# barrust/pyprobables

Hardware: AMD Instinct MI355X
Metric: million keys/sec insert+lookup (Bloom m=2^28 k=7, CMS 2^20x5) (higher is better)
Workload: dtype u64; 1 GPU; cfg2 Bloom m=2^28 k=7: per rank per step clear + insert 10M 16B keys + (merge) + check them; keys_per_rank=10000000, key_bytes=16, m_bits=268435456, k=7, parallelism=single GPU

## Files before the change

pyprobables_amd/csrc/psk_capi.hip:

```cpp
#include "psk_host.hpp"

#include <map>
#include <mutex>
#include <utility>

static thread_local char g_err[512] = "";

int fail(int code, const char *fmt, ...)
{
    va_list ap;
    va_start(ap, fmt);
    vsnprintf(g_err, sizeof(g_err), fmt, ap);
    va_end(ap);
    return code;
}


extern "C" const char *psk_last_error(void) { return g_err; }
extern "C" int psk_version(void) { return 100; }

extern "C" int psk_device_count(int *count)
{
    if (!count) return fail(PSK_EINVAL, "count is NULL");
    int n = 0;
// ... 444 lines not shown
    s->opt[d->ho] = value;
    return PSK_OK;
}

extern "C" int psk_sketch_get_option(psk_sketch *s, const char *name, int64_t *value)
{
    if (!s || !name || !value) return fail(PSK_EINVAL, "NULL argument");
    if (!strcmp(name, "table_private")) {
        *value = s->table_private ? 1 : 0;
        return PSK_OK;
    }
    if (!strcmp(name, "window_pending_batches")) {
        *value = s->win.n ? (int64_t)s->win.batches.size() : 0;
        return PSK_OK;
    }
    const OptDesc *d = opt_find(name);
    if (!d || d->ho < 0) return fail(PSK_EINVAL, "%s is not a per-sketch option", name);
    *value = s->opt[d->ho] != kHoUnset ? s->opt[d->ho] : __atomic_load_n(d->var, __ATOMIC_RELAXED);
    return PSK_OK;
}

extern "C" int psk_get_option(const char *name, int64_t *value)
{
    if (!name || !value) return fail(PSK_EINVAL, "NULL argument");
    const OptDesc *d = opt_find(name);
    if (!d) return fail(PSK_EINVAL, "unknown option %s", name);
    *value = __atomic_load_n(d->var, __ATOMIC_RELAXED);
    return PSK_OK;
}

// ... 33 lines not shown
```

pyprobables_amd/csrc/psk_host.hpp:

```cpp
#pragma once
#include "psk_device.hpp"
#include "psk_partition.hpp"
#include "psk_part_bins.hpp"

#include <hip/hip_runtime.h>

#include <cstdarg>
#include <cstdio>
#include <cstdlib>
#include <cstring>
#include <new>
#include <type_traits>
#include <vector>

#include "../../include/psk.h"

using namespace psk;

#define PSK_HIDDEN __attribute__((visibility("hidden")))

PSK_HIDDEN int fail(int code, const char *fmt, ...);

#define HIP_TRY(expr)                                                                                   \
    do {                                                                                                \
// ... 201 lines not shown
                               uint64_t max_buckets = kPartMaxBuckets, int target_lg = 8)
{
    if (cells >= (1ULL << 32) || cells < (1ULL << 16)) return false;
    const uint32_t lg = 63 - __builtin_clzll(cells);
    int shift = (int)lg - target_lg;
    if (shift > (int)max_shift) shift = max_shift;
    if (shift < (int)min_shift) shift = min_shift;
    const uint64_t B = (cells + (1ULL << shift) - 1) >> shift;
    if (B > max_buckets) return false;
    g->nbuckets = (uint32_t)B;
    g->shift = (uint32_t)shift;
    g->dbg = (uint32_t)g_part_debug | (g_ragged_sort == 0 ? kGeomNoSortBit : 0u);
    g->split = g->split_idx = 0;
    g->dense = 0;
    g->append = 0;
    return true;
}

static inline bool nib_geometry(uint64_t cells, bool update, PartGeom *g)
{
    if (update ? cells <= (1ULL << g_nib_min_lg_update) : cells < (1ULL << g_nib_min_lg_lookup)) return false;
    return part_slices(cells, kNibShift, 15, g, kPartMaxBuckets, 8);
}

static inline bool nib_load_ok(uint64_t n, uint32_t k, uint64_t cells) { return n * (uint64_t)k * 2 <= cells * 5; }

static inline bool scat_geometry(const psk_sketch *s, uint64_t cap, PartGeom *g)
{
    if (!nib_geometry(s->m, true, g)) return false;
    g->k = s->k;
// ... 101 lines not shown
        tk = ((n + nwg * tiles_per_wg - 1) / (nwg * tiles_per_wg) + 63) & ~63ULL;
        if (tk > tile_full) tk = tile_full;
    }
    const double mean = (double)tiles_per_wg * (double)tk * kk / (double)g->nbuckets;
    uint64_t segcap = (uint64_t)(mean / 6.0 + 0.5 * (double)tiles_per_wg + 8.0 * __builtin_sqrt(mean) / 6.0 + 16.0);
    if constexpr (pay_tile_tag<Pay>::value) {
        if (tiles_per_wg > 16) return fail(PSK_EINVAL, "lookup round of %llu keys needs %llu tiles per workgroup (max 16)",
                                           (unsigned long long)n, (unsigned long long)tiles_per_wg);
    }
    if (segcap >= (1u << 24) || (uint64_t)g->nbuckets * segcap >= (1ULL << 32))
        return fail(PSK_EINVAL, "partition round of %llu keys is too large (segments of %llu groups)", (unsigned long long)n, (unsigned long long)segcap);
    g->nwg = (uint32_t)nwg;
    g->segcap = (uint32_t)segcap;
    g->tile = (uint32_t)tk;
    g->dense = (mean / 6.0 + 0.5 * (double)tiles_per_wg) < (double)g_part_dense_groups ? 1u : 0u;
    PSK_TRY(ensure(s->s_part, (uint64_t)g->nbuckets * nwg * segcap * 16 + 256));
    PSK_TRY(ensure(s->s_cnt, (uint64_t)g->nbuckets * nwg * 4 + 128));
    auto kern = k_part_bins<Src, IdxFn, Pay, Spill, KT, kBinKpt>;
    PSK_TRY(set_dyn_lds(kern, bp.lds));
    hipLaunchKernelGGL(kern, dim3((unsigned)nwg), dim3(kBinThreads), bp.lds, st, src, idxfn, pay, spill, *g, (uint32_t)n, bp.cap, bp.stride,
                       (uint32_t *)s->s_cnt.p, (uint4 *)s->s_part.p);
    HIP_TRY(hipGetLastError());
    return PSK_OK;
}
template <class Src, class IdxFn, class Pay, class Spill, int KT, int NT>
static int launch_scatter_nt(psk_sketch *s, const Src &src, const IdxFn &idxfn, const Pay &pay, const Spill &spill, PartGeom *g,
                             uint64_t n, hipStream_t st, uint32_t want_wgs, const ScatterTarget *fixed = nullptr)
{
    if constexpr (bins_eligible<Src, Pay, KT>::value) {
        BinsPlan bp;
// ... 40 lines not shown
        if (tk > tile_full) tk = tile_full;
    }
    const size_t lds = scatter_lds_bytes<Pay, KT, NT>(g, tk, kSorted);
    const double mean = (double)tiles_per_wg * (double)tk * kk / (double)g->nbuckets;
    uint64_t segcap = (uint64_t)(mean / Tile::GS + 0.5 * (double)tiles_per_wg + 8.0 * __builtin_sqrt(mean) / Tile::GS + 16.0);
    if constexpr (Pay::mode == kModeKeyed || pay_tile_tag<Pay>::value) {
        if (tiles_per_wg > 16) return fail(PSK_EINVAL, "lookup round of %llu keys needs %llu tiles per workgroup (max 16)",
                                           (unsigned long long)n, (unsigned long long)tiles_per_wg);
    }
    if (segcap >= (1u << 24) || (uint64_t)g->nbuckets * segcap >= (1ULL << 32))
        return fail(PSK_EINVAL, "partition round of %llu keys is too large (segments of %llu groups)", (unsigned long long)n, (unsigned long long)segcap);
    g->nwg = (uint32_t)nwg;
    g->segcap = (uint32_t)segcap;
    g->tile = (uint32_t)tk;
    g->dense = (mean / Tile::GS + 0.5 * (double)tiles_per_wg) < (double)g_part_dense_groups ? 1u : 0u;
    PSK_TRY(ensure(s->s_part, (uint64_t)g->nbuckets * nwg * segcap * 16 + 256));
    PSK_TRY(ensure(s->s_cnt, (uint64_t)g->nbuckets * nwg * 4 + 128));
    auto kern = k_part_scatter<Src, IdxFn, Pay, Spill, KT, NT>;
    PSK_TRY(set_dyn_lds(kern, lds));
    hipLaunchKernelGGL(kern, dim3((unsigned)nwg), dim3(NT), lds, st, src, idxfn, pay, spill, *g, n, (uint32_t *)s->s_cnt.p,
                       (uint4 *)s->s_part.p);
    HIP_TRY(hipGetLastError());
    return PSK_OK;
}


template <class Pay, int KT, bool FAT = true>
static int scatter_threads(const PartGeom *g)
{
    if constexpr (!FAT && (pay_fat512<Pay>::value || pay_fat1024<Pay>::value)) return scatter_threads<PaySlim<Pay>, KT, false>(g);
// ... 233 lines not shown
```

pyprobables_amd/csrc/psk_part_bins.hpp:

```cpp
#pragma once
#include "psk_partition.hpp"

namespace psk {

#ifndef PSK_BINS_NT
#define PSK_BINS_NT 768
#endif
constexpr int kBinThreads = PSK_BINS_NT;
constexpr int kBinMinWaves = kBinThreads <= 512 ? 4 : (kBinThreads <= 768 ? 6 : 8);
#ifndef PSK_BINS_KPT
#define PSK_BINS_KPT 2
#endif
constexpr int kBinKpt = PSK_BINS_KPT;
constexpr int kBinSlicesPerLane = 2;

template <class Pay>
struct pay_bins_ok { static constexpr bool value = false; };
template <>
struct pay_bins_ok<PayNone> { static constexpr bool value = true; };
template <>
struct pay_bins_ok<PayTileTag> { static constexpr bool value = true; };
template <>
struct pay_bins_ok<PayWeightSmall> { static constexpr bool value = true; };

constexpr uint32_t kBinHead = 2;
template <bool WP>
__device__ __forceinline__ uint4 bin_short_group(const uint2 a0, const uint2 a1, const uint2 a2, uint32_t nv, uint32_t mask, uint32_t t0, uint32_t t1)
{
    uint32_t f[6] = {a0.x, a0.y, a1.x, a1.y, a2.x, a2.y};
#pragma unroll
    for (int x = 1; x < 6; ++x)
        if ((uint32_t)x >= nv) f[x] = WP ? 0u : mask;
    const uint32_t n0 = nv < 3u ? nv : 3u, n1 = nv - n0;
    uint4 o;
    o.x = f[0] | (f[1] << 20);
    o.y = (f[1] >> 12) | (f[2] << 8) | ((n0 | t0) << 28);
    o.z = f[3] | (f[4] << 20);
    o.w = (f[4] >> 12) | (f[5] << 8) | ((n1 | t1) << 28);
    return o;
}
template <class Src, class IdxFn, class Pay, class Spill, int KT, int KPT>
__global__ __launch_bounds__(kBinThreads, kBinMinWaves) void k_part_bins(Src src, IdxFn idxfn, Pay pay, Spill spill, PartGeom g, uint32_t n, uint32_t cap,
                                                              uint32_t stride, uint32_t *segcnt, uint4 *buckets)
{
    constexpr int NT = kBinThreads;
    extern __shared__ __attribute__((aligned(16))) uint32_t smem[];
    char *lds = reinterpret_cast<char *>(smem);
    const uint32_t B = g.nbuckets;
    constexpr bool kExactK = KT != 8;
    const uint32_t k = kExactK ? (uint32_t)KT : g.k;
    const uint32_t mask = (1u << g.shift) - 1;
    const uint32_t tk = g.tile;
    const uint32_t ntiles = (n + tk - 1) / tk;
    const uint32_t last = n ? n - 1 : 0;
    const uint32_t stride4 = stride * 4u;
    const uint32_t lg_slices = 31u - (uint32_t)__builtin_clz(B);
    const uint32_t full4 = (cap + kBinHead) * 4u;
    constexpr uint32_t kCnt = 4;

    uint32_t L = 1;
    while (2 * L * B <= (uint32_t)NT) L *= 2;
    constexpr int kSlicesPerLane = kBinSlicesPerLane;
    const uint32_t sub = B <= (uint32_t)NT ? threadIdx.x % L : 0u;
    uint32_t myb[kSlicesPerLane], cur[kSlicesPerLane];
    uint32_t carry[kSlicesPerLane];
    uint4 *seg[kSlicesPerLane];
// ... 160 lines not shown
            const uint32_t ngroups = whole + (tail ? 1u : 0u);
            uint2 *e = reinterpret_cast<uint2 *>(bin + kBinHead * 4u);
            uint4 *out = seg[s] + cur[s];
            if (cur[s] + ngroups <= g.segcap) {
                const uint32_t hi0 = (3u | t0) << 28, hi1 = (3u | t1) << 28;
                for (uint32_t gq = sub; gq < whole; gq += L) {
                    const uint2 a0 = e[3 * gq], a1 = e[3 * gq + 1], a2 = e[3 * gq + 2];
                    uint4 o;
                    o.x = a0.x | (a0.y << 20);
                    o.y = (a0.y >> 12) | (a1.x << 8) | hi0;
                    o.z = a1.y | (a2.x << 20);
                    o.w = (a2.x >> 12) | (a2.y << 8) | hi1;
                    if (!(dbg & 1)) out[gq] = o;
                }
                if constexpr (pay_tile_tag<Pay>::value) {
                    if (tail && sub == 0 && !(dbg & 1)) out[0] = bin_short_group<WP>(e[0], e[1], e[2], rem, mask, t0, t1);
                }
                if (rem && whole && sub == (whole & (L - 1))) {
                    __builtin_amdgcn_wave_barrier();
                    const uint2 a0 = e[3 * whole], a1 = e[3 * whole + 1], a2 = e[3 * whole + 2];
                    e[0] = a0;
                    e[1] = a1;
                    e[2] = a2;
                }
                carry[s] = tail ? 0u : rem;
                cur[s] += ngroups;
            } else {
                const uint32_t nall = whole + (rem ? 1u : 0u);
                for (uint32_t gq = sub; gq < nall; gq += L) {
                    const uint2 a0 = e[3 * gq], a1 = e[3 * gq + 1], a2 = e[3 * gq + 2];
                    const uint32_t left = c - 6u * gq, nv = left < 6u ? left : 6u;
                    if (cur[s] + gq < g.segcap) {
                        out[gq] = bin_short_group<WP>(a0, a1, a2, nv, mask, t0, t1);
                    } else {
                        const uint32_t f[6] = {a0.x, a0.y, a1.x, a1.y, a2.x, a2.y};
#pragma unroll
                        for (int x = 0; x < 6; ++x)
                            if ((uint32_t)x < nv) {
                                if constexpr (pay_tile_tag<Pay>::value) {
                                    spill((b << g.shift) | f[x], tile);
                                    if (ordinal) spill((b << g.shift) | f[x], tile - gridDim.x);
                                } else if constexpr (WP) spill((b << g.shift) | (f[x] & mask), f[x] >> 15);
                                else spill((b << g.shift) | f[x], 0u);
                            }
                    }
                }
                carry[s] = 0;
                cur[s] += nall;
// ... 7 lines not shown
            Src::pin(kcur[q]);
            if constexpr (WP) asm volatile("" : "+v"(wcur[q]));
        }
        PSK_BIN_TICK(2);
        lds_barrier();
        PSK_BIN_TICK(3);
    }
    if (ordinal != ~0u) {
        const uint32_t t0 = pay_tile_tag<Pay>::value ? (ordinal & 3u) << 2 : 0u, t1 = pay_tile_tag<Pay>::value ? ordinal & 12u : 0u;
#pragma unroll
        for (int s = 0; s < kSlicesPerLane; ++s) {
            if (myb[s] == ~0u || sub != 0 || carry[s] == 0) continue;
            const uint2 *e = reinterpret_cast<const uint2 *>(lds + myb[s] * stride4 + kBinHead * 4u);
            const uint2 a0 = e[0], a1 = e[1], a2 = e[2];
            if (cur[s] < g.segcap) {
                if (!(dbg & 1)) seg[s][cur[s]] = bin_short_group<WP>(a0, a1, a2, carry[s], mask, t0, t1);
            } else {
                const uint32_t f[6] = {a0.x, a0.y, a1.x, a1.y, a2.x, a2.y};
#pragma unroll
                for (int x = 0; x < 6; ++x)
                    if ((uint32_t)x < carry[s]) {
                        if constexpr (pay_tile_tag<Pay>::value) spill((myb[s] << g.shift) | f[x], ordinal * gridDim.x + blockIdx.x);
                        else if constexpr (WP) spill((myb[s] << g.shift) | (f[x] & mask), f[x] >> 15);
                        else spill((myb[s] << g.shift) | f[x], 0u);
                    }
            }
            cur[s] += 1;
        }
    }
    if (t_lane) {
        unsigned long long *prof = reinterpret_cast<unsigned long long *>(segcnt + (size_t)g.nbuckets * g.nwg);
// ... 33 lines not shown
```

pyprobables_amd/csrc/psk_part_bloom_check.hip:

```cpp
#include "psk_host.hpp"
#include "psk_lookup.hpp"

static inline uint32_t keyed_wgs(const PartGeom &g) { return g.nbuckets >= 2048 ? 1024u : 0u; }

static int check_round_scatter(psk_sketch *s, const Batch &sub, uint64_t cnt, uint8_t *out, uint32_t *defer, PartGeom *g,
                               hipStream_t st, bool *handled)
{
    return with_part_source(sub, handled, [&](auto src) {
        using Src = decltype(src);
        return with_kt<Src>(s->k, [&](auto kt) {
            constexpr int KT = decltype(kt)::value;
            SpillBloomTest spill{(const uint32_t *)s->table, out, defer};
            return launch_scatter<Src, IdxBloom<kTuPow2>, PayKeyId, SpillBloomTest, KT>(s, src, IdxBloom<kTuPow2>{s->md}, PayKeyId{},
                                                                                         spill, g, cnt, st, keyed_wgs(*g));
        });
    });
}

static int check_round_test(psk_sketch *s, const PartGeom &g, uint8_t *out, hipStream_t st, unsigned long long *miss_ctr = nullptr)
{
    const size_t lds = (size_t)1 << (g.shift - 3);
    PSK_TRY(set_dyn_lds(k_bloom_test, lds));
    hipLaunchKernelGGL(k_bloom_test, dim3(g.nbuckets), dim3(kApplyThreads), lds, st, (const uint32_t *)s->table, s->padded_bytes / 4, g,
                       (const uint32_t *)s->s_cnt.p, (const uint4 *)s->s_part.p, out, miss_ctr);
// ... 106 lines not shown
                    }
                }
                s->tflag_wgs = want;
                return (int)PSK_OK;
            });
        }) != PSK_OK || !handled || cap == 0) return false;
    if (round_keys > cap) {
        const uint64_t rounds = (b.n + cap - 1) / cap;
        round_keys = ((b.n + rounds - 1) / rounds + 4095) & ~4095ULL;
        if (round_keys > cap) round_keys = cap;
    }
    *round_keys_out = round_keys;
    return true;
}

static uint32_t *tflag_base(psk_sketch *s) { return (uint32_t *)s->s_tflag.p + 4; }
constexpr uint32_t kResolveWgs = 256;

static int tile_flag_scatter(psk_sketch *s, const Batch &sub, uint64_t cnt, bool defer, PartGeom *g, uint32_t *gen_out, hipStream_t st, bool *handled)
{
    return with_part_source(sub, handled, [&](auto src) {
        using Src = decltype(src);
        return with_kt<Src>(s->k, [&](auto kt) {
            constexpr int KT = decltype(kt)::value;
            const uint64_t flag_bytes = (cnt / 64 + 2048) * 4 + 16;
            if (flag_bytes > s->s_tflag.cap || s->tflag_gen == 0xFFFFFFFFu) {
                PSK_TRY(ensure(s->s_tflag, flag_bytes));
                HIP_TRY(hipMemsetAsync(s->s_tflag.p, 0, s->s_tflag.cap, st));
                s->tflag_gen = 0;
            }
            const uint32_t gen = ++s->tflag_gen;
            *gen_out = gen;
            SpillBloomFlag spill{(const uint32_t *)s->table, tflag_base(s), gen, defer ? 1u : 0u};
            return launch_scatter<Src, IdxBloom<kTuPow2>, PayTileTag, SpillBloomFlag, KT>(s, src, IdxBloom<kTuPow2>{s->md}, PayTileTag{}, spill, g, cnt, st,
                                                                                          s->tflag_wgs);
        });
    });
}

static int tile_flag_test(psk_sketch *s, const Batch &sub, uint64_t cnt, const PartGeom &g, uint32_t gen, uint8_t *out, unsigned long long publish_units, hipStream_t st)
{
    bool handled = false;
    PSK_TRY(with_part_source(sub, &handled, [&](auto src) {
        using Src = decltype(src);
        uint32_t *tflag = tflag_base(s);
        const size_t lds = (size_t)1 << (g.shift - 3);
        PSK_TRY(set_dyn_lds(k_bloom_test_flag, lds));
        hipLaunchKernelGGL(k_bloom_test_flag, dim3(g.nbuckets), dim3(kApplyThreads), lds, st, (const uint32_t *)s->table, s->padded_bytes / 4, g,
                           (const uint32_t *)s->s_cnt.p, (const uint4 *)s->s_part.p, tflag, gen, s->lk.dev, out, cnt);
        HIP_TRY(hipGetLastError());
        const uint64_t ntiles = (cnt + g.tile - 1) / g.tile;
        LookupPublish pub;
        if (publish_units && s->eff[HO_BLOOM_LOOKUP] == 2 && s->lk.dev) pub = LookupPublish{s->lk.dev, s->lk.pin, publish_units, 3};
        hipLaunchKernelGGL((k_bloom_flag_resolve<Src, kTuPow2>), dim3((unsigned)(ntiles < kResolveWgs ? ntiles : kResolveWgs)), dim3(kResolveThreads), 0, st, src,
                           (const uint32_t *)s->table, s->md, s->k, (const uint32_t *)tflag, gen, g.tile, cnt, out, pub);
        HIP_TRY(hipGetLastError());
        return (int)PSK_OK;
    }));
    return handled ? (int)PSK_OK : fail(PSK_EHIP, "tile-flag lookup: layout lost its partitioned instantiation");
}

static int bloom_check_tile_flags(psk_sketch *s, const Batch &b, uint8_t *out_dev, hipStream_t st, bool *done)
{
    *done = false;
    PartGeom g;
    uint64_t round_keys = 0;
    if (!tile_flag_geometry(s, b, &g, &round_keys)) return PSK_OK;
    for (uint64_t start = 0; start < b.n; start += round_keys) {
// ... 74 lines not shown
            else
                hipLaunchKernelGGL((k_bloom_check_lazy<Src, true, false>), grid, block, 0, st, src, (const uint32_t *)s->table, s->md, s->k, b.n, out_dev, ctr);
        } else {
            hipLaunchKernelGGL((k_bloom_check_lazy<Src, false, false>), grid, block, 0, st, src, (const uint32_t *)s->table, s->md, s->k, b.n, out_dev, ctr);
        }
        HIP_TRY(hipGetLastError());
        return (int)PSK_OK;
    }));
    *done = handled;
    return PSK_OK;
}

static int choose_scheme(psk_sketch *s, hipStream_t st)
{
    if (s->eff[HO_BLOOM_LOOKUP] != 2) return (int)s->eff[HO_BLOOM_LOOKUP];
    if (!s->lk.dev) {
        HIP_TRY(hipMalloc((void **)&s->lk.dev, 8));
        void *pin = nullptr;
        HIP_TRY(hipHostMalloc(&pin, 64, hipHostMallocDefault));
        s->lk.pin = (volatile unsigned long long *)pin;
        for (int e = 0; e < 8; ++e) s->lk.pin[e] = 0;
        HIP_TRY(hipMemsetAsync(s->lk.dev, 0, 8, st));
    }
    const unsigned long long miss = s->lk.pin[0], units = s->lk.pin[1], by = s->lk.pin[2], seq = s->lk.pin[3];
    if (units) {
        const double f = (double)miss / (double)units;
        const bool clean_call = by == 1 ? f == 0.0 : f <= 1e-6;
        if (seq != s->lk.seen_seq) {
            s->lk.seen_seq = seq;
            s->lk.clean = clean_call ? s->lk.clean + 1 : 0;
        }
        const bool flags_ok = clean_call && s->lk.clean >= 2;
        const double kLazyStay = s->m <= (1ULL << 29) ? 1.6 : (s->m <= (1ULL << 30) ? 2.2 : 3.0);
        const double kLazyEnter = s->m <= (1ULL << 29) ? 0.93 : (s->m <= (1ULL << 30) ? 0.85 : 0.72);
        constexpr uint32_t kLazyBackoff = 32;
        volatile unsigned long long &lazy_seq = s->lk.pin[4], &lazy_wait = s->lk.pin[5];
        if (seq != lazy_seq) {
            lazy_seq = seq;
// ... 124 lines not shown
```

pyprobables_amd/csrc/psk_partition.hpp:

```cpp
#pragma once
#include <type_traits>
#include "psk_device.hpp"

#ifndef PSK_BENCH_KNOBS
#define PSK_BENCH_KNOBS 0
#endif

namespace psk {

constexpr bool kBenchKnobs = PSK_BENCH_KNOBS != 0;
constexpr int kPartThreads = 512;
constexpr int kPartProbes = 32;
constexpr int kPartMaxBuckets = 2048;
constexpr int kPartScanPerThread = 4;
constexpr bool kPartPipeline = true;
constexpr bool kPartHash32 = true;
constexpr uint32_t kNibShift = 18;
constexpr uint32_t kGeomNoSortBit = 0x40000000u;
constexpr int kSortSub = 16;
constexpr int kSortBins = 64 * kSortSub;
constexpr uint32_t kPadProbe = 0xFFFFFFFFu;
#ifndef PSK_EXP_PRIO
#define PSK_EXP_PRIO 1
#endif

enum PartMode { kModePlain = 0, kModeInline = 1, kModeKeyed = 2 };

struct PartGeom {
    uint32_t nbuckets;
    uint32_t shift;
    uint32_t nwg;
    uint32_t segcap;
    uint32_t k;
    uint32_t tile;
    uint32_t dbg;
    uint32_t split;
    uint32_t split_idx;
    uint32_t dense;
    uint32_t append;
};

__device__ __forceinline__ uint64_t seg_index(const PartGeom &g, uint32_t b, uint32_t wg) { return (uint64_t)wg * g.nbuckets + b; }

template <bool POW2>
struct IdxBloom {
    static constexpr bool lo32 = POW2 && kPartHash32;
    Mod md;
    __device__ __forceinline__ uint32_t operator()(uint32_t, uint64_t h) const
    {
        return POW2 ? (uint32_t)reduce<true>(md, h) : reduce_small(md, h);
    }
    __device__ __forceinline__ uint32_t from32(uint32_t, uint32_t h) const { return h & (uint32_t)md.mask; }
};
template <bool POW2>
// ... 243 lines not shown
struct SpillBloomFlag {
    const uint32_t *tab;
    uint32_t *tileflag;
    uint32_t gen;
    uint32_t defer;
    __device__ __forceinline__ void operator()(uint32_t idx, uint32_t tile) const
    {
        if (defer || ((tab[idx >> 5] >> (idx & 31)) & 1u) == 0) {
            tileflag[tile] = gen;
            tileflag[-1] = gen;
        }
    }
};

__device__ __forceinline__ void lds_barrier() { asm volatile("s_waitcnt lgkmcnt(0)\n\ts_barrier" ::: "memory"); }

__device__ __forceinline__ uint32_t wave_inclusive_scan(uint32_t x)
{
    x += (uint32_t)__builtin_amdgcn_update_dpp(0, (int)x, 0x111, 0xf, 0xf, false);
    x += (uint32_t)__builtin_amdgcn_update_dpp(0, (int)x, 0x112, 0xf, 0xf, false);
    x += (uint32_t)__builtin_amdgcn_update_dpp(0, (int)x, 0x114, 0xf, 0xf, false);
    x += (uint32_t)__builtin_amdgcn_update_dpp(0, (int)x, 0x118, 0xf, 0xf, false);
    x += (uint32_t)__builtin_amdgcn_update_dpp(0, (int)x, 0x142, 0xa, 0xf, false);
    x += (uint32_t)__builtin_amdgcn_update_dpp(0, (int)x, 0x143, 0xc, 0xf, false);
    return x;
}

template <int NT>
__device__ __forceinline__ uint32_t block_exclusive_scan(uint32_t v, uint32_t *wave_tot , uint32_t *total)
{
// ... 711 lines not shown
#pragma unroll
                for (int x = 0; x < GS; ++x)
                    if (v[x] != kPadProbe) spill((slice << g2.shift) | (v[x] & mask), v[x] >> g1.shift);
            }
        }
        __syncthreads();
    }
    if (threadIdx.x < S) {
        const uint32_t slice = (c << sub_bits) + threadIdx.x;
        if (slice < g2.nbuckets) segcnt2[(uint64_t)slice * g2.nwg + p] = cur[threadIdx.x] < g2.segcap ? cur[threadIdx.x] : g2.segcap;
    }
}

constexpr int kApplyThreads = 1024;
constexpr int kApplyWaves = kApplyThreads / 64;

__device__ __forceinline__ uint32_t lane_segment_count(const uint32_t *segcnt, const PartGeom &g, uint32_t b)
{
    const uint32_t lane = threadIdx.x & 63, wave = threadIdx.x >> 6;
    const uint32_t S = g.split > 1 ? g.split : 1, s0 = g.split > 1 ? g.split_idx : 0;
    const uint32_t mine_total = g.nwg > s0 ? (g.nwg - s0 + S - 1) / S : 0;
    const uint32_t nseg = mine_total > wave ? (mine_total - wave + kApplyWaves - 1) / kApplyWaves : 0;
    return lane < nseg ? segcnt[(uint64_t)b * g.nwg + s0 + S * (wave + kApplyWaves * lane)] : 0u;
}

template <int D, class Body>
__device__ __forceinline__ void for_each_batch_at(const uint4 *buckets, const uint32_t *segcnt, const PartGeom &g, uint32_t b,
                                                  const uint4 pad, Body body, uint32_t mycnt_pre = ~0u)
{
    const uint32_t lane = threadIdx.x & 63, wave = threadIdx.x >> 6;
    const uint32_t S = g.split > 1 ? g.split : 1, s0 = g.split > 1 ? g.split_idx : 0;
    const uint32_t mycnt = mycnt_pre != ~0u ? mycnt_pre : lane_segment_count(segcnt, g, b);
    if (g.dense) {
        const uint32_t incl = wave_inclusive_scan(mycnt), excl = incl - mycnt;
        const uint32_t T = (uint32_t)__builtin_amdgcn_readlane((int)incl, 63);
        for (uint32_t G0 = 0; G0 < T; G0 += 64u * D) {
            uint4 q[D];
            uint64_t at[D];
            uint32_t wg[D];
#pragma unroll
            for (int d = 0; d < D; ++d) {
// ... 12 lines not shown
                }
                seg = seg < 64 ? seg : 63;
                wg[d] = s0 + S * (wave + kApplyWaves * seg);
                q[d] = pad;
                at[d] = ~0ULL;
                if (G < T) {
                    const uint64_t idx = seg_index(g, b, wg[d]) * g.segcap + (G - first);
                    q[d] = buckets[idx];
                    at[d] = idx;
                }
            }
            body(q, at, wg);
        }
        return;
    }
    const uint32_t chunks = (mycnt + 63) >> 6;
    const uint32_t incl = wave_inclusive_scan(chunks), excl = incl - chunks;
    const uint32_t C = (uint32_t)__builtin_amdgcn_readlane((int)incl, 63);
    for (uint32_t c0 = 0; c0 < C; c0 += D) {
        uint4 q[D];
        uint64_t at[D];
        uint32_t wg[D];
#pragma unroll
        for (int d = 0; d < D; ++d) {
            const uint32_t cc = c0 + d;
            const uint32_t seg = (uint32_t)__builtin_popcountll(__ballot(incl <= cc));
            const uint32_t sl = seg < 64 ? seg : 63;
            const uint32_t v = (cc - (uint32_t)__builtin_amdgcn_readlane((int)excl, sl)) * 64 + lane;
            const uint32_t cnt = seg < 64 ? (uint32_t)__builtin_amdgcn_readlane((int)mycnt, sl) : 0;
            wg[d] = s0 + S * (wave + kApplyWaves * sl);
            const uint64_t base = seg_index(g, b, wg[d]) * g.segcap;
            q[d] = pad;
            at[d] = ~0ULL;
            if (v < cnt) {
                q[d] = buckets[base + v];
                at[d] = base + v;
            }
        }
        body(q, at, wg);
    }
}

template <int D, class Body>
__device__ __forceinline__ void for_each_batch(const uint4 *buckets, const uint32_t *segcnt, const PartGeom &g, uint32_t b,
                                               const uint4 pad, Body body)
{
    const uint32_t lane = threadIdx.x & 63, wave = threadIdx.x >> 6;
    const uint32_t nseg = g.nwg > wave ? (g.nwg - wave + kApplyWaves - 1) / kApplyWaves : 0;
    uint32_t mycnt = 0;
    if (lane < nseg) mycnt = segcnt[(uint64_t)b * g.nwg + wave + kApplyWaves * lane];
    if (g.dense) {
        const uint32_t incl = wave_inclusive_scan(mycnt), excl = incl - mycnt;
        const uint32_t T = (uint32_t)__builtin_amdgcn_readlane((int)incl, 63);
        for (uint32_t G0 = 0; G0 < T; G0 += 64u * D) {
            uint4 q[D];
#pragma unroll
            for (int d = 0; d < D; ++d) {
                const uint32_t row = G0 + 64u * (uint32_t)d;
// ... 5 lines not shown
                for (; t < 64; ++t) {
                    const uint32_t end_t = (uint32_t)__builtin_amdgcn_readlane((int)incl, t);
                    if (end_t > row + 63u) break;
                    const bool past = G >= end_t;
                    seg = past ? t + 1 : seg;
                    first = past ? end_t : first;
                }
                seg = seg < 64 ? seg : 63;
                q[d] = pad;
                if (G < T) q[d] = buckets[seg_index(g, b, wave + kApplyWaves * seg) * g.segcap + (G - first)];
            }
            body(q);
        }
        return;
    }
    const uint32_t chunks = (mycnt + 63) >> 6;
    const uint32_t incl = wave_inclusive_scan(chunks), excl = incl - chunks;
    const uint32_t C = (uint32_t)__builtin_amdgcn_readlane((int)incl, 63);
    for (uint32_t c0 = 0; c0 < C; c0 += D) {
        uint4 q[D];
#pragma unroll
        for (int d = 0; d < D; ++d) {
            const uint32_t cc = c0 + d;
            const uint32_t seg = (uint32_t)__builtin_popcountll(__ballot(incl <= cc));
            const uint32_t sl = seg < 64 ? seg : 63;
            const uint32_t v = (cc - (uint32_t)__builtin_amdgcn_readlane((int)excl, sl)) * 64 + lane;
            const uint32_t cnt = seg < 64 ? (uint32_t)__builtin_amdgcn_readlane((int)mycnt, sl) : 0;
            const uint4 *src = buckets + seg_index(g, b, wave + kApplyWaves * sl) * g.segcap;
            q[d] = pad;
            if (v < cnt) q[d] = src[v];
        }
        body(q);
    }
}

constexpr int kApplyDepth = 12;

constexpr uint64_t kNtTableWords = 1ULL << 25;
__device__ __forceinline__ uint4 slice_piece(const uint32_t *tab, uint64_t tab_words, uint64_t w0, uint32_t w, bool nt = false)
{
    const uint64_t gw = w0 + w;
    if (gw + 3 < tab_words) {
        if (nt) {
            typedef unsigned int nt_u32x4 __attribute__((ext_vector_type(4)));
            const nt_u32x4 v = __builtin_nontemporal_load(reinterpret_cast<const nt_u32x4 *>(tab + gw));
// ... 15 lines not shown
    for (uint32_t wb = threadIdx.x * 4; wb < slice_words; wb += kApplyThreads * 4 * kSliceLoads) {
        uint4 t[kSliceLoads];
#pragma unroll
        for (int u = 0; u < kSliceLoads; ++u) {
            const uint32_t w = wb + (uint32_t)u * kApplyThreads * 4;
            t[u] = w < slice_words ? slice_piece(tab, tab_words, w0, w, nt) : make_uint4(0, 0, 0, 0);
        }
#pragma unroll
        for (int u = 0; u < kSliceLoads; ++u) {
            const uint32_t w = wb + (uint32_t)u * kApplyThreads * 4;
            if (w < slice_words) *reinterpret_cast<uint4 *>(smem + w) = t[u];
        }
    }
}

template <int DEPTH = kApplyDepth, class F4>
__device__ __forceinline__ void for_each_group(const uint4 *buckets, const uint32_t *segcnt, const PartGeom &g, uint32_t b,
                                               const uint4 pad, F4 f4)
{
    for_each_batch<DEPTH>(buckets, segcnt, g, b, pad, [&](const uint4 (&q)[DEPTH]) {
#pragma unroll
        for (int d = 0; d < DEPTH; ++d) f4(q[d]);
    });
}

template <class Pre, class Post>
__device__ __forceinline__ void for_each_group_padded(const uint4 *buckets, const uint32_t *segcnt, const PartGeom &g, uint32_t b,
                                                      const uint4 pad, Pre pre, Post post)
{
    for_each_batch<kApplyDepth>(buckets, segcnt, g, b, pad, [&](const uint4 (&q)[kApplyDepth]) {
        uint4 w[kApplyDepth];
#pragma unroll
        for (int d = 0; d < kApplyDepth; ++d) w[d] = pre(q[d]);
#pragma unroll
        for (int d = 0; d < kApplyDepth; ++d) post(q[d], w[d]);
// ... 4 lines not shown
constexpr uint32_t kBloomApplyCtrSpilled = 7;
struct BloomApplyStore {
    uint32_t on = 0;
    const uint32_t *spill = nullptr;
    uint32_t spill_cap = 0;
    long long *ctr = nullptr;
};
static __global__ __launch_bounds__(kApplyThreads) void k_bloom_apply(uint32_t *tab, uint64_t tab_words, PartGeom g,
                                                               const uint32_t *segcnt, const uint4 *buckets, BloomApplyStore sm)
{
    extern __shared__ __attribute__((aligned(16))) uint32_t smem[];
    const uint32_t b = blockIdx.x;
    const uint32_t slice_words = 1u << (g.shift - 5);
    for (uint32_t w = threadIdx.x; w < slice_words; w += kApplyThreads) smem[w] = 0;
    __syncthreads();
    auto half = [&](uint32_t lo, uint32_t hi) {
        const unsigned long long h = ((unsigned long long)hi << 32) | lo;
        const uint32_t nv = hi >> 28;
        if (nv > 0) { const uint32_t x = (uint32_t)h & 0xFFFFFu; atomicOr(&smem[x >> 5], 1u << (x & 31)); }
        if (nv > 1) { const uint32_t x = (uint32_t)(h >> 20) & 0xFFFFFu; atomicOr(&smem[x >> 5], 1u << (x & 31)); }
        if (nv > 2) { const uint32_t x = (uint32_t)(h >> 40) & 0xFFFFFu; atomicOr(&smem[x >> 5], 1u << (x & 31)); }
    };
    for_each_group(buckets, segcnt, g, b, make_uint4(0, 0, 0, 0), [&](const uint4 q) { half(q.x, q.y); half(q.z, q.w); });
    uint32_t spilled = 0;
    if (sm.on) {
        spilled = sm.spill[0];
        const uint32_t nsp = spilled < sm.spill_cap ? spilled : sm.spill_cap;
        const uint32_t lmask = (1u << g.shift) - 1u;
        for (uint32_t i = threadIdx.x; i < nsp; i += kApplyThreads) {
            const uint32_t x = sm.spill[2 + i];
            if ((x >> g.shift) == b) atomicOr(&smem[(x & lmask) >> 5], 1u << (x & 31));
        }
    }
    __syncthreads();
    const uint64_t w0 = (uint64_t)b * slice_words;
    const bool nt = tab_words >= kNtTableWords;
    typedef unsigned int nt_u32x4 __attribute__((ext_vector_type(4)));
    if (sm.on) {
// ... 72 lines not shown
static __global__ __launch_bounds__(kApplyThreads) void k_bloom_test(const uint32_t *tab, uint64_t tab_words, PartGeom g,
                                                              const uint32_t *segcnt, const uint4 *buckets, uint8_t *out,
                                                              unsigned long long *miss_ctr)
{
    uint32_t nmiss = 0;
    extern __shared__ __attribute__((aligned(16))) uint32_t smem[];
    const uint32_t b = blockIdx.x;
    const uint32_t slice_words = 1u << (g.shift - 5);
    const uint32_t mask = (1u << g.shift) - 1;
    const uint64_t w0 = (uint64_t)b * slice_words;
    const uint32_t dbg = kBenchKnobs ? g.dbg : 0u;
    const uint32_t mycnt = lane_segment_count(segcnt, g, b);
    if (!(dbg & 128)) load_slice(smem, tab, tab_words, w0, slice_words);
    __syncthreads();
    const uint32_t kmask = (1u << (31 - g.shift)) - 1;
    for_each_batch_at<kApplyDepth>(buckets, segcnt, g, b, make_uint4(0, 0, 0, 0), [&](const uint4 (&q)[kApplyDepth], const uint64_t (&at)[kApplyDepth],
                                                                                     const uint32_t (&wg)[kApplyDepth]) {
        uint4 w[kApplyDepth];
#pragma unroll
        for (int d = 0; d < kApplyDepth; ++d) {
            if (dbg & 64) { w[d] = make_uint4(~0u, ~0u, ~0u, ~0u); continue; }
            w[d] = make_uint4(smem[(q[d].x & mask) >> 5], smem[(q[d].y & mask) >> 5], smem[(q[d].z & mask) >> 5], smem[(q[d].w & mask) >> 5]);
        }
#pragma unroll
        for (int d = 0; d < kApplyDepth; ++d) {
            const bool live = at[d] != ~0ULL;
            const bool mx = live && ((w[d].x >> (q[d].x & 31)) & 1u) == 0;
            const bool my = live && ((w[d].y >> (q[d].y & 31)) & 1u) == 0;
            const bool mz = live && ((w[d].z >> (q[d].z & 31)) & 1u) == 0;
            const bool mw = live && ((w[d].w >> (q[d].w & 31)) & 1u) == 0;
            nmiss += (uint32_t)mx + (uint32_t)my + (uint32_t)mz + (uint32_t)mw;
            if (mx | my | mz | mw) {
                const uint32_t ordinal = (q[d].x >> 31) | ((q[d].y >> 31) << 1) | ((q[d].z >> 31) << 2) | ((q[d].w >> 31) << 3);
                const uint32_t kbase = (ordinal * g.nwg + wg[d]) * g.tile;
                if (mx) out[kbase + ((q[d].x >> g.shift) & kmask)] = 0;
                if (my) out[kbase + ((q[d].y >> g.shift) & kmask)] = 0;
                if (mz) out[kbase + ((q[d].z >> g.shift) & kmask)] = 0;
// ... 32 lines not shown
            uint4 *mid = reinterpret_cast<uint4 *>(out + (m0 - a0));
            for (uint64_t i = lo + threadIdx.x; i < hi; i += kApplyThreads) mid[i] = ones;
            if (b == 0) {
                if (threadIdx.x < (uint32_t)(m0 - a0)) out[threadIdx.x] = 1;
                if (threadIdx.x < (uint32_t)(a1 - m1)) out[(m1 - a0) + threadIdx.x] = 1;
            }
        } else if (b == 0) {
            for (uint64_t i = threadIdx.x; i < n; i += kApplyThreads) out[i] = 1;
        }
    }
    const uint32_t slice_words = 1u << (g.shift - 5);
    const uint64_t w0 = (uint64_t)b * slice_words;
    const uint32_t mycnt = lane_segment_count(segcnt, g, b);
    load_slice(smem, tab, tab_words, w0, slice_words);
    __syncthreads();
    for_each_batch_at<kFlagDepth>(buckets, segcnt, g, b, make_uint4(0, 0, 0, 0), [&](const uint4 (&q)[kFlagDepth], const uint64_t (&)[kFlagDepth],
                                                                                   const uint32_t (&wg)[kFlagDepth]) {
        uint32_t f[kFlagDepth][6], w[kFlagDepth][6];
#pragma unroll
        for (int d = 0; d < kFlagDepth; ++d) {
            f[d][0] = q[d].x & 0xFFFFFu;
            f[d][1] = __builtin_amdgcn_alignbit(q[d].y, q[d].x, 20) & 0xFFFFFu;
            f[d][2] = (q[d].y >> 8) & 0xFFFFFu;
            f[d][3] = q[d].z & 0xFFFFFu;
            f[d][4] = __builtin_amdgcn_alignbit(q[d].w, q[d].z, 20) & 0xFFFFFu;
            f[d][5] = (q[d].w >> 8) & 0xFFFFFu;
#pragma unroll
            for (int e = 0; e < 6; ++e) w[d][e] = smem[f[d][e] >> 5];
        }
#pragma unroll
        for (int d = 0; d < kFlagDepth; ++d) {
            uint32_t clear = 0;
#pragma unroll
            for (int e = 0; e < 6; ++e) clear |= (((w[d][e] >> (f[d][e] & 31)) & 1u) ^ 1u) << e;
            const uint32_t n0 = (q[d].y >> 28) & 3u, n1 = (q[d].w >> 28) & 3u;
            const uint32_t valid = ((1u << n0) - 1u) | (((1u << n1) - 1u) << 3);
            clear &= valid;
            if (clear) {
                nmiss += (uint32_t)__builtin_popcount(clear);
                const uint32_t ordinal = (q[d].y >> 30) | ((q[d].w >> 30) << 2);
                tileflag[ordinal * g.nwg + wg[d]] = gen;
                if (ordinal) tileflag[(ordinal - 1u) * g.nwg + wg[d]] = gen;
                tileflag[-1] = gen;
            }
        }
    }, mycnt);
    if (miss_ctr) {
        for (int o = 32; o > 0; o >>= 1) nmiss += __shfl_down(nmiss, o);
        __syncthreads();
        if ((threadIdx.x & 63) == 0) smem[threadIdx.x >> 6] = nmiss;
        __syncthreads();
        if (threadIdx.x == 0) {
            unsigned long long t = 0;
            for (int w = 0; w < kApplyWaves; ++w) t += smem[w];
            if (t) atomicAdd(miss_ctr, t);
        }
    }
}

constexpr int kResolveThreads = 1024;
struct LookupPublish {
// ... 218 lines not shown
```

Before: 61130 Mkeys/s.

## Pad short Bloom groups with duplicate fields and use raw LDS addressing in apply/flag kernels

Short partitioned groups are now padded by repeating their first valid field instead of a masked sentinel when the geometry flag allows it. This lets the bloom OR and flag-check kernels apply all six fields branch-free and test membership with a single AND across the fields, skipping per-field validity masks. LDS accesses are rewritten as raw address-space-3 byte offsets, with a trap that asserts dynamic LDS starts at zero, and wave indices are made scalar via readfirstlane to simplify segment base addressing. Lookup tally allocation is also made unconditional so miss counts are always published and exposed as a queryable option, which adds a small allocation and publish cost.

```diff
diff --git a/pyprobables_amd/csrc/psk_capi.hip b/pyprobables_amd/csrc/psk_capi.hip
--- a/pyprobables_amd/csrc/psk_capi.hip
+++ b/pyprobables_amd/csrc/psk_capi.hip
@@ -482,6 +482,10 @@
         *value = s->win.n ? (int64_t)s->win.batches.size() : 0;
         return PSK_OK;
     }
+    if (!strcmp(name, "bloom_lookup_misses")) {
+        *value = s->lk.pin && s->lk.pin[1] ? (int64_t)s->lk.pin[0] : -1;
+        return PSK_OK;
+    }
     const OptDesc *d = opt_find(name);
     if (!d || d->ho < 0) return fail(PSK_EINVAL, "%s is not a per-sketch option", name);
     *value = s->opt[d->ho] != kHoUnset ? s->opt[d->ho] : __atomic_load_n(d->var, __ATOMIC_RELAXED);
diff --git a/pyprobables_amd/csrc/psk_host.hpp b/pyprobables_amd/csrc/psk_host.hpp
--- a/pyprobables_amd/csrc/psk_host.hpp
+++ b/pyprobables_amd/csrc/psk_host.hpp
@@ -239,6 +239,7 @@
     g->split = g->split_idx = 0;
     g->dense = 0;
     g->append = 0;
+    g->dup_pads = 0;
     return true;
 }
 
@@ -370,6 +371,7 @@
     g->segcap = (uint32_t)segcap;
     g->tile = (uint32_t)tk;
     g->dense = (mean / 6.0 + 0.5 * (double)tiles_per_wg) < (double)g_part_dense_groups ? 1u : 0u;
+    g->dup_pads = (std::is_same<Pay, PayNone>::value && std::is_same<Spill, SpillBloomOr>::value) || pay_tile_tag<Pay>::value ? 1u : 0u;
     PSK_TRY(ensure(s->s_part, (uint64_t)g->nbuckets * nwg * segcap * 16 + 256));
     PSK_TRY(ensure(s->s_cnt, (uint64_t)g->nbuckets * nwg * 4 + 128));
     auto kern = k_part_bins<Src, IdxFn, Pay, Spill, KT, kBinKpt>;
@@ -440,6 +442,7 @@
     g->segcap = (uint32_t)segcap;
     g->tile = (uint32_t)tk;
     g->dense = (mean / Tile::GS + 0.5 * (double)tiles_per_wg) < (double)g_part_dense_groups ? 1u : 0u;
+    g->dup_pads = 0;
     PSK_TRY(ensure(s->s_part, (uint64_t)g->nbuckets * nwg * segcap * 16 + 256));
     PSK_TRY(ensure(s->s_cnt, (uint64_t)g->nbuckets * nwg * 4 + 128));
     auto kern = k_part_scatter<Src, IdxFn, Pay, Spill, KT, NT>;
diff --git a/pyprobables_amd/csrc/psk_part_bins.hpp b/pyprobables_amd/csrc/psk_part_bins.hpp
--- a/pyprobables_amd/csrc/psk_part_bins.hpp
+++ b/pyprobables_amd/csrc/psk_part_bins.hpp
@@ -25,12 +25,13 @@
 
 constexpr uint32_t kBinHead = 2;
 template <bool WP>
-__device__ __forceinline__ uint4 bin_short_group(const uint2 a0, const uint2 a1, const uint2 a2, uint32_t nv, uint32_t mask, uint32_t t0, uint32_t t1)
+__device__ __forceinline__ uint4 bin_short_group(const uint2 a0, const uint2 a1, const uint2 a2, uint32_t nv, uint32_t mask, uint32_t t0, uint32_t t1, bool dup)
 {
     uint32_t f[6] = {a0.x, a0.y, a1.x, a1.y, a2.x, a2.y};
+    const uint32_t fill = WP ? 0u : (dup ? f[0] : mask);
 #pragma unroll
     for (int x = 1; x < 6; ++x)
-        if ((uint32_t)x >= nv) f[x] = WP ? 0u : mask;
+        if ((uint32_t)x >= nv) f[x] = fill;
     const uint32_t n0 = nv < 3u ? nv : 3u, n1 = nv - n0;
     uint4 o;
     o.x = f[0] | (f[1] << 20);
@@ -50,6 +51,7 @@
     constexpr bool kExactK = KT != 8;
     const uint32_t k = kExactK ? (uint32_t)KT : g.k;
     const uint32_t mask = (1u << g.shift) - 1;
+    const bool dup = g.dup_pads != 0;
     const uint32_t tk = g.tile;
     const uint32_t ntiles = (n + tk - 1) / tk;
     const uint32_t last = n ? n - 1 : 0;
@@ -240,7 +242,7 @@
                     if (!(dbg & 1)) out[gq] = o;
                 }
                 if constexpr (pay_tile_tag<Pay>::value) {
-                    if (tail && sub == 0 && !(dbg & 1)) out[0] = bin_short_group<WP>(e[0], e[1], e[2], rem, mask, t0, t1);
+                    if (tail && sub == 0 && !(dbg & 1)) out[0] = bin_short_group<WP>(e[0], e[1], e[2], rem, mask, t0, t1, dup);
                 }
                 if (rem && whole && sub == (whole & (L - 1))) {
                     __builtin_amdgcn_wave_barrier();
@@ -257,7 +259,7 @@
                     const uint2 a0 = e[3 * gq], a1 = e[3 * gq + 1], a2 = e[3 * gq + 2];
                     const uint32_t left = c - 6u * gq, nv = left < 6u ? left : 6u;
                     if (cur[s] + gq < g.segcap) {
-                        out[gq] = bin_short_group<WP>(a0, a1, a2, nv, mask, t0, t1);
+                        out[gq] = bin_short_group<WP>(a0, a1, a2, nv, mask, t0, t1, dup);
                     } else {
                         const uint32_t f[6] = {a0.x, a0.y, a1.x, a1.y, a2.x, a2.y};
 #pragma unroll
@@ -295,7 +297,7 @@
             const uint2 *e = reinterpret_cast<const uint2 *>(lds + myb[s] * stride4 + kBinHead * 4u);
             const uint2 a0 = e[0], a1 = e[1], a2 = e[2];
             if (cur[s] < g.segcap) {
-                if (!(dbg & 1)) seg[s][cur[s]] = bin_short_group<WP>(a0, a1, a2, carry[s], mask, t0, t1);
+                if (!(dbg & 1)) seg[s][cur[s]] = bin_short_group<WP>(a0, a1, a2, carry[s], mask, t0, t1, dup);
             } else {
                 const uint32_t f[6] = {a0.x, a0.y, a1.x, a1.y, a2.x, a2.y};
 #pragma unroll
diff --git a/pyprobables_amd/csrc/psk_part_bloom_check.hip b/pyprobables_amd/csrc/psk_part_bloom_check.hip
--- a/pyprobables_amd/csrc/psk_part_bloom_check.hip
+++ b/pyprobables_amd/csrc/psk_part_bloom_check.hip
@@ -144,6 +144,18 @@
     return true;
 }
 
+static int ensure_lookup_tally(psk_sketch *s, hipStream_t st)
+{
+    if (s->lk.dev) return PSK_OK;
+    HIP_TRY(hipMalloc((void **)&s->lk.dev, 8));
+    void *pin = nullptr;
+    HIP_TRY(hipHostMalloc(&pin, 64, hipHostMallocDefault));
+    s->lk.pin = (volatile unsigned long long *)pin;
+    for (int e = 0; e < 8; ++e) s->lk.pin[e] = 0;
+    HIP_TRY(hipMemsetAsync(s->lk.dev, 0, 8, st));
+    return PSK_OK;
+}
+
 static uint32_t *tflag_base(psk_sketch *s) { return (uint32_t *)s->s_tflag.p + 4; }
 constexpr uint32_t kResolveWgs = 256;
 
@@ -171,6 +183,7 @@
 static int tile_flag_test(psk_sketch *s, const Batch &sub, uint64_t cnt, const PartGeom &g, uint32_t gen, uint8_t *out, unsigned long long publish_units, hipStream_t st)
 {
     bool handled = false;
+    PSK_TRY(ensure_lookup_tally(s, st));
     PSK_TRY(with_part_source(sub, &handled, [&](auto src) {
         using Src = decltype(src);
         uint32_t *tflag = tflag_base(s);
@@ -181,7 +194,7 @@
         HIP_TRY(hipGetLastError());
         const uint64_t ntiles = (cnt + g.tile - 1) / g.tile;
         LookupPublish pub;
-        if (publish_units && s->eff[HO_BLOOM_LOOKUP] == 2 && s->lk.dev) pub = LookupPublish{s->lk.dev, s->lk.pin, publish_units, 3};
+        if (publish_units && s->lk.dev && s->lk.pin) pub = LookupPublish{s->lk.dev, s->lk.pin, publish_units, 3};
         hipLaunchKernelGGL((k_bloom_flag_resolve<Src, kTuPow2>), dim3((unsigned)(ntiles < kResolveWgs ? ntiles : kResolveWgs)), dim3(kResolveThreads), 0, st, src,
                            (const uint32_t *)s->table, s->md, s->k, (const uint32_t *)tflag, gen, g.tile, cnt, out, pub);
         HIP_TRY(hipGetLastError());
@@ -286,14 +299,7 @@
 static int choose_scheme(psk_sketch *s, hipStream_t st)
 {
     if (s->eff[HO_BLOOM_LOOKUP] != 2) return (int)s->eff[HO_BLOOM_LOOKUP];
-    if (!s->lk.dev) {
-        HIP_TRY(hipMalloc((void **)&s->lk.dev, 8));
-        void *pin = nullptr;
-        HIP_TRY(hipHostMalloc(&pin, 64, hipHostMallocDefault));
-        s->lk.pin = (volatile unsigned long long *)pin;
-        for (int e = 0; e < 8; ++e) s->lk.pin[e] = 0;
-        HIP_TRY(hipMemsetAsync(s->lk.dev, 0, 8, st));
-    }
+    PSK_TRY(ensure_lookup_tally(s, st));
     const unsigned long long miss = s->lk.pin[0], units = s->lk.pin[1], by = s->lk.pin[2], seq = s->lk.pin[3];
     if (units) {
         const double f = (double)miss / (double)units;
diff --git a/pyprobables_amd/csrc/psk_partition.hpp b/pyprobables_amd/csrc/psk_partition.hpp
--- a/pyprobables_amd/csrc/psk_partition.hpp
+++ b/pyprobables_amd/csrc/psk_partition.hpp
@@ -38,6 +38,7 @@
     uint32_t split_idx;
     uint32_t dense;
     uint32_t append;
+    uint32_t dup_pads;
 };
 
 __device__ __forceinline__ uint64_t seg_index(const PartGeom &g, uint32_t b, uint32_t wg) { return (uint64_t)wg * g.nbuckets + b; }
@@ -311,6 +312,18 @@
 };
 
 __device__ __forceinline__ void lds_barrier() { asm volatile("s_waitcnt lgkmcnt(0)\n\ts_barrier" ::: "memory"); }
+
+typedef __attribute__((address_space(3))) uint32_t lds_u32_t;
+__device__ __forceinline__ void lds_image_at_zero()
+{
+    if (__builtin_amdgcn_groupstaticsize() != 0) __builtin_trap();
+}
+__device__ __forceinline__ uint32_t lds_word_at(uint32_t byte_off) { return *reinterpret_cast<const lds_u32_t *>(byte_off); }
+__device__ __forceinline__ void lds_or_at(uint32_t byte_off, uint32_t bits)
+{
+    (void)__hip_atomic_fetch_or(reinterpret_cast<lds_u32_t *>(byte_off), bits, __ATOMIC_RELAXED, __HIP_MEMORY_SCOPE_WORKGROUP);
+}
+__device__ __forceinline__ uint32_t lds_word_of_bit(uint32_t x) { return (x >> 3) & 0x1FFFCu; }
 
 __device__ __forceinline__ uint32_t wave_inclusive_scan(uint32_t x)
 {
@@ -1052,6 +1065,7 @@
 
 constexpr int kApplyThreads = 1024;
 constexpr int kApplyWaves = kApplyThreads / 64;
+__device__ __forceinline__ uint32_t wave_uniform() { return (uint32_t)__builtin_amdgcn_readfirstlane((int)(threadIdx.x >> 6)); }
 
 __device__ __forceinline__ uint32_t lane_segment_count(const uint32_t *segcnt, const PartGeom &g, uint32_t b)
 {
@@ -1062,7 +1076,7 @@
     return lane < nseg ? segcnt[(uint64_t)b * g.nwg + s0 + S * (wave + kApplyWaves * lane)] : 0u;
 }
 
-template <int D, class Body>
+template <int D, bool SBASE = false, class Body>
 __device__ __forceinline__ void for_each_batch_at(const uint4 *buckets, const uint32_t *segcnt, const PartGeom &g, uint32_t b,
                                                   const uint4 pad, Body body, uint32_t mycnt_pre = ~0u)
 {
@@ -1105,6 +1119,7 @@
         }
         return;
     }
+    const uint32_t wave_s = SBASE ? wave_uniform() : wave;
     const uint32_t chunks = (mycnt + 63) >> 6;
     const uint32_t incl = wave_inclusive_scan(chunks), excl = incl - chunks;
     const uint32_t C = (uint32_t)__builtin_amdgcn_readlane((int)incl, 63);
@@ -1119,12 +1134,14 @@
             const uint32_t sl = seg < 64 ? seg : 63;
             const uint32_t v = (cc - (uint32_t)__builtin_amdgcn_readlane((int)excl, sl)) * 64 + lane;
             const uint32_t cnt = seg < 64 ? (uint32_t)__builtin_amdgcn_readlane((int)mycnt, sl) : 0;
-            wg[d] = s0 + S * (wave + kApplyWaves * sl);
+            wg[d] = s0 + S * (wave_s + kApplyWaves * sl);
             const uint64_t base = seg_index(g, b, wg[d]) * g.segcap;
+            const char *src = reinterpret_cast<const char *>(buckets + base);
             q[d] = pad;
             at[d] = ~0ULL;
             if (v < cnt) {
-                q[d] = buckets[base + v];
+                if constexpr (SBASE) q[d] = *reinterpret_cast<const uint4 *>(src + (v << 4));
+                else q[d] = buckets[base + v];
                 at[d] = base + v;
             }
         }
@@ -1132,7 +1149,7 @@
     }
 }
 
-template <int D, class Body>
+template <int D, bool SBASE = false, class Body>
 __device__ __forceinline__ void for_each_batch(const uint4 *buckets, const uint32_t *segcnt, const PartGeom &g, uint32_t b,
                                                const uint4 pad, Body body)
 {
@@ -1168,6 +1185,7 @@
         }
         return;
     }
+    const uint32_t wave_s = SBASE ? wave_uniform() : wave;
     const uint32_t chunks = (mycnt + 63) >> 6;
     const uint32_t incl = wave_inclusive_scan(chunks), excl = incl - chunks;
     const uint32_t C = (uint32_t)__builtin_amdgcn_readlane((int)incl, 63);
@@ -1180,9 +1198,12 @@
             const uint32_t sl = seg < 64 ? seg : 63;
             const uint32_t v = (cc - (uint32_t)__builtin_amdgcn_readlane((int)excl, sl)) * 64 + lane;
             const uint32_t cnt = seg < 64 ? (uint32_t)__builtin_amdgcn_readlane((int)mycnt, sl) : 0;
-            const uint4 *src = buckets + seg_index(g, b, wave + kApplyWaves * sl) * g.segcap;
+            const uint4 *src = buckets + seg_index(g, b, wave_s + kApplyWaves * sl) * g.segcap;
             q[d] = pad;
-            if (v < cnt) q[d] = src[v];
+            if (v < cnt) {
+                if constexpr (SBASE) q[d] = *reinterpret_cast<const uint4 *>(reinterpret_cast<const char *>(src) + (v << 4));
+                else q[d] = src[v];
+            }
         }
         body(q);
     }
@@ -1228,11 +1249,11 @@
     }
 }
 
-template <int DEPTH = kApplyDepth, class F4>
+template <int DEPTH = kApplyDepth, bool SBASE = false, class F4>
 __device__ __forceinline__ void for_each_group(const uint4 *buckets, const uint32_t *segcnt, const PartGeom &g, uint32_t b,
                                                const uint4 pad, F4 f4)
 {
-    for_each_batch<DEPTH>(buckets, segcnt, g, b, pad, [&](const uint4 (&q)[DEPTH]) {
+    for_each_batch<DEPTH, SBASE>(buckets, segcnt, g, b, pad, [&](const uint4 (&q)[DEPTH]) {
 #pragma unroll
         for (int d = 0; d < DEPTH; ++d) f4(q[d]);
     });
@@ -1267,14 +1288,30 @@
     const uint32_t slice_words = 1u << (g.shift - 5);
     for (uint32_t w = threadIdx.x; w < slice_words; w += kApplyThreads) smem[w] = 0;
     __syncthreads();
+    lds_image_at_zero();
     auto half = [&](uint32_t lo, uint32_t hi) {
-        const unsigned long long h = ((unsigned long long)hi << 32) | lo;
         const uint32_t nv = hi >> 28;
-        if (nv > 0) { const uint32_t x = (uint32_t)h & 0xFFFFFu; atomicOr(&smem[x >> 5], 1u << (x & 31)); }
-        if (nv > 1) { const uint32_t x = (uint32_t)(h >> 20) & 0xFFFFFu; atomicOr(&smem[x >> 5], 1u << (x & 31)); }
-        if (nv > 2) { const uint32_t x = (uint32_t)(h >> 40) & 0xFFFFFu; atomicOr(&smem[x >> 5], 1u << (x & 31)); }
+        const uint32_t x0 = lo, x1 = __builtin_amdgcn_alignbit(hi, lo, 20), x2 = hi >> 8;
+        if (nv > 0) lds_or_at(lds_word_of_bit(x0), 1u << (x0 & 31));
+        if (nv > 1) lds_or_at(lds_word_of_bit(x1), 1u << (x1 & 31));
+        if (nv > 2) lds_or_at(lds_word_of_bit(x2), 1u << (x2 & 31));
     };
-    for_each_group(buckets, segcnt, g, b, make_uint4(0, 0, 0, 0), [&](const uint4 q) { half(q.x, q.y); half(q.z, q.w); });
+    if (g.dup_pads) {
+        for_each_group<kApplyDepth, true>(buckets, segcnt, g, b, make_uint4(0, 0, 0, 0), [&](const uint4 q) {
+            if (q.y & 0x30000000u) {
+                const uint32_t x1 = __builtin_amdgcn_alignbit(q.y, q.x, 20), x2 = q.y >> 8;
+                const uint32_t x4 = __builtin_amdgcn_alignbit(q.w, q.z, 20), x5 = q.w >> 8;
+                lds_or_at(lds_word_of_bit(q.x), 1u << (q.x & 31));
+                lds_or_at(lds_word_of_bit(x1), 1u << (x1 & 31));
+                lds_or_at(lds_word_of_bit(x2), 1u << (x2 & 31));
+                lds_or_at(lds_word_of_bit(q.z), 1u << (q.z & 31));
+                lds_or_at(lds_word_of_bit(x4), 1u << (x4 & 31));
+                lds_or_at(lds_word_of_bit(x5), 1u << (x5 & 31));
+            }
+        });
+    } else {
+        for_each_group<kApplyDepth, true>(buckets, segcnt, g, b, make_uint4(0, 0, 0, 0), [&](const uint4 q) { half(q.x, q.y); half(q.z, q.w); });
+    }
     uint32_t spilled = 0;
     if (sm.on) {
         spilled = sm.spill[0];
@@ -1377,13 +1414,16 @@
     if (!(dbg & 128)) load_slice(smem, tab, tab_words, w0, slice_words);
     __syncthreads();
     const uint32_t kmask = (1u << (31 - g.shift)) - 1;
-    for_each_batch_at<kApplyDepth>(buckets, segcnt, g, b, make_uint4(0, 0, 0, 0), [&](const uint4 (&q)[kApplyDepth], const uint64_t (&at)[kApplyDepth],
+    lds_image_at_zero();
+    const uint32_t wmask4 = (mask >> 5) << 2;
+    for_each_batch_at<kApplyDepth, true>(buckets, segcnt, g, b, make_uint4(0, 0, 0, 0), [&](const uint4 (&q)[kApplyDepth], const uint64_t (&at)[kApplyDepth],
                                                                                      const uint32_t (&wg)[kApplyDepth]) {
         uint4 w[kApplyDepth];
 #pragma unroll
         for (int d = 0; d < kApplyDepth; ++d) {
             if (dbg & 64) { w[d] = make_uint4(~0u, ~0u, ~0u, ~0u); continue; }
-            w[d] = make_uint4(smem[(q[d].x & mask) >> 5], smem[(q[d].y & mask) >> 5], smem[(q[d].z & mask) >> 5], smem[(q[d].w & mask) >> 5]);
+            w[d] = make_uint4(lds_word_at((q[d].x >> 3) & wmask4), lds_word_at((q[d].y >> 3) & wmask4), lds_word_at((q[d].z >> 3) & wmask4),
+                              lds_word_at((q[d].w >> 3) & wmask4));
         }
 #pragma unroll
         for (int d = 0; d < kApplyDepth; ++d) {
@@ -1446,37 +1486,67 @@
     const uint32_t mycnt = lane_segment_count(segcnt, g, b);
     load_slice(smem, tab, tab_words, w0, slice_words);
     __syncthreads();
-    for_each_batch_at<kFlagDepth>(buckets, segcnt, g, b, make_uint4(0, 0, 0, 0), [&](const uint4 (&q)[kFlagDepth], const uint64_t (&)[kFlagDepth],
-                                                                                   const uint32_t (&wg)[kFlagDepth]) {
-        uint32_t f[kFlagDepth][6], w[kFlagDepth][6];
-#pragma unroll
-        for (int d = 0; d < kFlagDepth; ++d) {
-            f[d][0] = q[d].x & 0xFFFFFu;
-            f[d][1] = __builtin_amdgcn_alignbit(q[d].y, q[d].x, 20) & 0xFFFFFu;
-            f[d][2] = (q[d].y >> 8) & 0xFFFFFu;
-            f[d][3] = q[d].z & 0xFFFFFu;
-            f[d][4] = __builtin_amdgcn_alignbit(q[d].w, q[d].z, 20) & 0xFFFFFu;
-            f[d][5] = (q[d].w >> 8) & 0xFFFFFu;
-#pragma unroll
-            for (int e = 0; e < 6; ++e) w[d][e] = smem[f[d][e] >> 5];
-        }
-#pragma unroll
-        for (int d = 0; d < kFlagDepth; ++d) {
-            uint32_t clear = 0;
-#pragma unroll
-            for (int e = 0; e < 6; ++e) clear |= (((w[d][e] >> (f[d][e] & 31)) & 1u) ^ 1u) << e;
-            const uint32_t n0 = (q[d].y >> 28) & 3u, n1 = (q[d].w >> 28) & 3u;
-            const uint32_t valid = ((1u << n0) - 1u) | (((1u << n1) - 1u) << 3);
-            clear &= valid;
-            if (clear) {
-                nmiss += (uint32_t)__builtin_popcount(clear);
-                const uint32_t ordinal = (q[d].y >> 30) | ((q[d].w >> 30) << 2);
-                tileflag[ordinal * g.nwg + wg[d]] = gen;
-                if (ordinal) tileflag[(ordinal - 1u) * g.nwg + wg[d]] = gen;
-                tileflag[-1] = gen;
-            }
-        }
-    }, mycnt);
+    lds_image_at_zero();
+    auto fields = [](const uint4 q, uint32_t (&x)[6]) {
+        x[0] = q.x;
+        x[1] = __builtin_amdgcn_alignbit(q.y, q.x, 20);
+        x[2] = q.y >> 8;
+        x[3] = q.z;
+        x[4] = __builtin_amdgcn_alignbit(q.w, q.z, 20);
+        x[5] = q.w >> 8;
+    };
+    auto judge = [&](const uint4 q, uint32_t wgd, const uint32_t (&x)[6], const uint32_t (&w)[6]) {
+        uint32_t clear = 0;
+#pragma unroll
+        for (int e = 0; e < 6; ++e) clear |= (((w[e] >> (x[e] & 31)) & 1u) ^ 1u) << e;
+        const uint32_t n0 = (q.y >> 28) & 3u, n1 = (q.w >> 28) & 3u;
+        const uint32_t valid = ((1u << n0) - 1u) | (((1u << n1) - 1u) << 3);
+        clear &= valid;
+        if (clear) {
+            nmiss += (uint32_t)__builtin_popcount(clear);
+            const uint32_t ordinal = (q.y >> 30) | ((q.w >> 30) << 2);
+            tileflag[ordinal * g.nwg + wgd] = gen;
+            if (ordinal) tileflag[(ordinal - 1u) * g.nwg + wgd] = gen;
+            tileflag[-1] = gen;
+        }
+    };
+    if (g.dup_pads) {
+        for_each_batch_at<kFlagDepth, true>(buckets, segcnt, g, b, make_uint4(0, 0, 0, 0), [&](const uint4 (&q)[kFlagDepth], const uint64_t (&)[kFlagDepth],
+                                                                                       const uint32_t (&wg)[kFlagDepth]) {
+            uint32_t w[kFlagDepth][6];
+#pragma unroll
+            for (int d = 0; d < kFlagDepth; ++d) {
+                uint32_t x[6];
+                fields(q[d], x);
+#pragma unroll
+                for (int e = 0; e < 6; ++e) w[d][e] = lds_word_at(lds_word_of_bit(x[e]));
+            }
+#pragma unroll
+            for (int d = 0; d < kFlagDepth; ++d) {
+                uint32_t x[6];
+                fields(q[d], x);
+                uint32_t all = ~0u;
+#pragma unroll
+                for (int e = 0; e < 6; ++e) all &= w[d][e] >> (x[e] & 31);
+                if (q[d].y & 0x30000000u) {
+                    if (!(all & 1u)) judge(q[d], wg[d], x, w[d]);
+                }
+            }
+        }, mycnt);
+    } else {
+        for_each_batch_at<kFlagDepth, true>(buckets, segcnt, g, b, make_uint4(0, 0, 0, 0), [&](const uint4 (&q)[kFlagDepth], const uint64_t (&)[kFlagDepth],
+                                                                                       const uint32_t (&wg)[kFlagDepth]) {
+            uint32_t x[kFlagDepth][6], w[kFlagDepth][6];
+#pragma unroll
+            for (int d = 0; d < kFlagDepth; ++d) {
+                fields(q[d], x[d]);
+#pragma unroll
+                for (int e = 0; e < 6; ++e) w[d][e] = lds_word_at(lds_word_of_bit(x[d][e]));
+            }
+#pragma unroll
+            for (int d = 0; d < kFlagDepth; ++d) judge(q[d], wg[d], x[d], w[d]);
+        }, mycnt);
+    }
     if (miss_ctr) {
         for (int o = 32; o > 0; o >>= 1) nmiss += __shfl_down(nmiss, o);
         __syncthreads();
```

After: 62830 Mkeys/s, median of 6. 1.03x the previous value.
